# certfhe/CSGN

Hardware: NVIDIA B200
Metric: ctxt-mul+decrypt output blocks/s (higher is better)
Workload: dtype u64

## Files before the change

csgn_b200/_native.py:

```python
import ctypes
import os
import re
import warnings

from . import build as _build

_u64 = ctypes.c_uint64
_u64p = ctypes.POINTER(ctypes.c_uint64)
_vp = ctypes.c_void_p
_vpp = ctypes.POINTER(ctypes.c_void_p)

SIGNATURES = {
    "csgn_init": (ctypes.c_int, [ctypes.c_int]),
    "csgn_shutdown": (ctypes.c_int, []),
    "csgn_is_initialized": (ctypes.c_int, []),
    "csgn_last_error": (ctypes.c_char_p, []),
    "csgn_version": (ctypes.c_char_p, []),
    "csgn_device_info": (ctypes.c_int, [ctypes.POINTER(ctypes.c_int), _u64p, _u64p, ctypes.POINTER(ctypes.c_int)]),
    "csgn_set_stream": (ctypes.c_int, [_vp]),
    "csgn_get_stream": (_vp, []),
    "csgn_set_auto_lanes": (ctypes.c_int, [ctypes.c_int]),
    "csgn_get_auto_lanes": (ctypes.c_int, []),
    "csgn_sync": (ctypes.c_int, []),
    "csgn_launch_count": (_u64, []),
    "csgn_words_per_block": (ctypes.c_uint32, [_u64]),
    "csgn_host_alloc": (ctypes.c_int, [ctypes.c_size_t, _vpp]),
    "csgn_host_free": (ctypes.c_int, [_vp]),
    "csgn_buf_upload": (ctypes.c_int, [_vp, _u64, ctypes.c_uint32, _vpp]),
    "csgn_buf_upload_copy": (ctypes.c_int, [_vp, _u64, ctypes.c_uint32, _vpp]),
    "csgn_buf_upload_batch": (ctypes.c_int, [_vp, _vp, ctypes.c_uint32, ctypes.c_uint32, _vp]),
    "csgn_buf_free_batch": (ctypes.c_int, [_vp, ctypes.c_uint32]),
    "csgn_buf_alloc": (ctypes.c_int, [_u64, ctypes.c_uint32, _vpp]),
    "csgn_buf_wrap": (ctypes.c_int, [_vp, _u64, ctypes.c_uint32, _vpp]),
    "csgn_buf_clone": (ctypes.c_int, [_vp, _vpp]),
    "csgn_buf_download": (ctypes.c_int, [_vp, _vp]),
    "csgn_buf_download_range": (ctypes.c_int, [_vp, _u64, _u64, _vp]),
    "csgn_buf_slice": (ctypes.c_int, [_vp, _u64, _u64, _vpp]),
    "csgn_buf_free": (ctypes.c_int, [_vp]),
    "csgn_buf_blocks": (_u64, [_vp]),
    "csgn_buf_words_per_block": (ctypes.c_uint32, [_vp]),
    "csgn_buf_device_ptr": (_vp, [_vp]),
    "csgn_mul": (ctypes.c_int, [_vp, _vp, _vpp]),
    "csgn_mul_into": (ctypes.c_int, [_vp, _vp, _vp]),
    "csgn_concat": (ctypes.c_int, [_vp, _vp, _vpp]),
    "csgn_append": (ctypes.c_int, [_vp, _vp]),
    "csgn_concat_lazy": (ctypes.c_int, [_vp, _vp, _vpp]),
    "csgn_buf_segments": (ctypes.c_int, [_vp]),
    "csgn_buf_retained": (ctypes.c_int, [_vp]),
    "csgn_buf_flatten": (ctypes.c_int, [_vp]),
    "csgn_key_create": (ctypes.c_int, [_u64, _vp, ctypes.c_uint32, _vpp]),
    "csgn_key_free": (ctypes.c_int, [_vp]),
    "csgn_decrypt": (ctypes.c_int, [_vp, _vp, ctypes.POINTER(ctypes.c_uint8)]),
    "csgn_decrypt_count": (ctypes.c_int, [_vp, _vp, _u64p]),
    "csgn_decrypt_count_async": (ctypes.c_int, [_vp, _vp, _vp]),
    "csgn_decrypt_product": (ctypes.c_int, [ctypes.POINTER(_vp), ctypes.c_uint32, _vp, ctypes.POINTER(ctypes.c_uint8), _u64p]),
    "csgn_decrypt_deferred": (ctypes.c_int, [_vp, _vp, _vpp]),
    "csgn_result_ready": (ctypes.c_int, [_vp]),
    "csgn_result_wait": (ctypes.c_int, [_vp, _u64p]),
    "csgn_result_free": (ctypes.c_int, [_vp]),
    "csgn_mul_count_async": (ctypes.c_int, [_vp, _vp, _vp, _vpp, _vp]),
    "csgn_mul_decrypt": (ctypes.c_int, [_vp, _vp, _vp, _vpp, ctypes.POINTER(ctypes.c_uint8), _u64p]),
    "csgn_mul_count_batch_async": (ctypes.c_int, [ctypes.POINTER(_vp), ctypes.POINTER(_vp), ctypes.c_uint32, _vp,
                                                  ctypes.POINTER(_vp), _vp]),
    "csgn_mul_decrypt_deferred": (ctypes.c_int, [_vp, _vp, _vp, _vpp, _vpp]),
    "csgn_mul_decrypt_sharded_async": (ctypes.c_int, [_vp, _vp, _vp, _vpp, _vp, ctypes.c_uint32, ctypes.c_uint32, _vp, _vp]),
    "csgn_mul_decrypt_sharded_batch_async": (ctypes.c_int, [ctypes.POINTER(_vp), ctypes.POINTER(_vp), ctypes.c_uint32, _vp,
                                                            ctypes.POINTER(_vp), _vp, ctypes.c_uint32, _vp]),
    "csgn_mul_batch": (ctypes.c_int, [ctypes.POINTER(_vp), ctypes.POINTER(_vp), ctypes.c_uint32, ctypes.POINTER(_vp)]),
    "csgn_mul_into_batch": (ctypes.c_int, [ctypes.POINTER(_vp), ctypes.POINTER(_vp), ctypes.c_uint32, ctypes.POINTER(_vp)]),
    "csgn_decrypt_count_batch_async": (ctypes.c_int, [ctypes.POINTER(_vp), ctypes.c_uint32, _vp, _vp]),
    "csgn_decrypt_batch": (ctypes.c_int, [ctypes.POINTER(_vp), ctypes.c_uint32, _vp, ctypes.POINTER(ctypes.c_uint8), _u64p]),
    "csgn_decrypt_sharded_batch_async": (ctypes.c_int, [ctypes.POINTER(_vp), ctypes.c_uint32, _vp, _vp, ctypes.c_uint32, _vp]),
    "csgn_decrypt_positions": (ctypes.c_int, [_vp, _u64, _vp, ctypes.c_uint32, ctypes.POINTER(ctypes.c_uint8)]),
    "csgn_encrypt_batch": (ctypes.c_int, [_vp, _vp, _u64, _u64, _u64, _vpp]),
    "csgn_seg_mul": (ctypes.c_int, [_vp, _vp, _vp, _vp, _u64, _vp, _vpp]),
    "csgn_seg_concat": (ctypes.c_int, [_vp, _vp, _vp, _vp, _u64, _vp, _vpp]),
    "csgn_seg_mul_sum": (ctypes.c_int, [ctypes.POINTER(_vp), ctypes.POINTER(_vp), ctypes.POINTER(_vp), ctypes.POINTER(_vp),
                                        ctypes.c_uint32, ctypes.POINTER(_vp), ctypes.POINTER(_vp), ctypes.c_uint32, _u64,
                                        _vp, _vpp]),
    "csgn_seg_mul_sum_compact": (ctypes.c_int, [ctypes.POINTER(_vp), ctypes.POINTER(_vp), ctypes.POINTER(_vp),
                                                ctypes.POINTER(_vp), ctypes.c_uint32, ctypes.POINTER(_vp),
                                                ctypes.POINTER(_vp), ctypes.c_uint32, _u64, ctypes.c_uint32, _vp, _vpp]),
# ... 87 lines not shown
```

csgn_b200/certfhe/device_types.cpp:

```cpp
#include "certFHE.h"
#include "engine_glue.h"

#include <cstdlib>
#include <ctime>
#include <utility>
#include <vector>

namespace certFHE {

namespace glue {

void check(int status, const char *what) {
    if (status != CSGN_OK) throw Error(string(what) + ": " + csgn_last_error());
}

void ensure_engine() {
    if (csgn_is_initialized()) return;
    check(csgn_init(-1), "csgn_init");
    check(csgn_set_auto_lanes(Library::getAutoLanes() ? 1 : 0), "csgn_set_auto_lanes");
}

}

namespace {

inline uint64_t canonical_bits(uint64_t i, uint64_t L, uint64_t rem) {
    return ((i % L) + 1 == L && rem) ? rem : 64;
}

void require_canonical_bitlen(const uint64_t *bitlen, uint64_t len, const Context &ctx) {
    const uint64_t L = ctx.getDefaultN(), rem = ctx.getN() % 64;
    uint64_t diff = 0;
    const uint64_t head = len < L ? len : L;
    for (uint64_t k = 0; k < head; ++k) diff |= bitlen[k] ^ canonical_bits(k, L, rem);
    if (len > L && memcmp(bitlen + L, bitlen, (size_t)(len - L) * sizeof(uint64_t)) != 0) diff = 1;
    if (!diff) return;
    for (uint64_t i = 0; i < len; ++i)
        if (bitlen[i] != canonical_bits(i, L, rem))
            throw Error("Ciphertext: bitlen[" + to_string(i) + "] = " + to_string(bitlen[i]) +
                        " is not the canonical pattern for N = " + to_string(ctx.getN()) +
                        " (the reference would mis-index such an object, src/SecretKey.cpp:133)");
}

uint64_t *copy_words(const uint64_t *src, uint64_t n) {
    uint64_t *p = new uint64_t[n ? n : 1];
    if (n) memcpy(p, src, n * sizeof(uint64_t));
    return p;
}

}

namespace {

std::shared_ptr<csgn_buf> adopt(csgn_buf *b) {
    return std::shared_ptr<csgn_buf>(b, [](csgn_buf *p) { csgn_buf_free(p); });
}

}

Ciphertext::Ciphertext()
    : certFHEcontext(nullptr), host_v(nullptr), host_bitlen(nullptr), host_len(0), host_v_valid(false),
      staged(false), sharded(false) {}

Ciphertext::Ciphertext(const uint64_t *V, const uint64_t *Bitlen, const uint64_t len, const Context &context)
    : Ciphertext() {
    certFHEcontext = new Context(context);
    const uint64_t L = context.getDefaultN();
    if (L == 0 || len % L != 0)
        throw Error("Ciphertext: len = " + to_string(len) + " is not a multiple of the " + to_string(L) +
                    " words per block");
    if (Bitlen) require_canonical_bitlen(Bitlen, len, context);
    glue::ensure_engine();
    csgn_buf *b = nullptr;
    glue::check(csgn_buf_upload_copy(V, len / L, (uint32_t)L, &b), "csgn_buf_upload_copy");
    dev = adopt(b);
}

Ciphertext::Ciphertext(const Ciphertext &o) : Ciphertext() {
    if (o.certFHEcontext) certFHEcontext = new Context(*o.certFHEcontext);
    sharded = o.sharded;
    if (o.staged) {
        host_v = copy_words(o.host_v, o.host_len);
        if (o.host_bitlen) host_bitlen = copy_words(o.host_bitlen, o.host_len);
        host_len = o.host_len;
        host_v_valid = true;
        staged = true;
    } else {
        dev = o.dev;
        factors = o.factors;
        product_slot = o.product_slot;
    }
}

Ciphertext::Ciphertext(Ciphertext &&o) noexcept
    : dev(std::move(o.dev)), factors(std::move(o.factors)), product_slot(std::move(o.product_slot)),
      certFHEcontext(o.certFHEcontext), host_v(o.host_v),
      host_bitlen(o.host_bitlen), host_len(o.host_len), host_v_valid(o.host_v_valid), staged(o.staged),
      sharded(o.sharded) {
    o.factors.clear();
    o.product_slot.reset();
    o.certFHEcontext = nullptr;
    o.host_v = o.host_bitlen = nullptr;
    o.host_len = 0;
    o.host_v_valid = o.staged = false;
}

Ciphertext::~Ciphertext() {
    release();
    delete certFHEcontext;
    certFHEcontext = nullptr;
}

void Ciphertext::invalidate_mirror() const {
    delete[] host_v;
    delete[] host_bitlen;
    host_v = host_bitlen = nullptr;
    host_len = 0;
    host_v_valid = false;
}

void Ciphertext::release() {
    dev.reset();
    factors.clear();
    product_slot.reset();
    invalidate_mirror();
    staged = false;
}
// ... 652 lines not shown
```

csgn_b200/csrc/capi.cu:

```cuda
#include "capi_internal.cuh"

#include <atomic>
#include <cstdarg>
#if defined(__x86_64__) && !defined(__CUDA_ARCH__)
#include <emmintrin.h>
#define CSGN_HAVE_SSE2_STREAM 1
#endif

#ifdef CSGN_BUILD_VARIANTS
#define CSGN_VERSION_STRING "csgn-b200 0.2 (sm_100a) +variants"
#else
#define CSGN_VERSION_STRING "csgn-b200 0.2 (sm_100a)"
#endif

namespace csgn {
namespace detail {

State g;
DeviceProps g_props;
std::atomic<uint64_t> g_launches{0};
thread_local std::string t_error;

int fail(int code, const char *fmt, ...) {
    char buf[512];
    va_list ap;
    va_start(ap, fmt);
    vsnprintf(buf, sizeof buf, fmt, ap);
    va_end(ap);
    t_error = buf;
    return code;
}

int cuda_fail(cudaError_t e, const char *what) {
    cudaGetLastError();
    return fail(e == cudaErrorMemoryAllocation ? CSGN_ERR_OUT_OF_MEMORY : CSGN_ERR_CUDA, "%s: %s (%s)", what,
                cudaGetErrorString(e), cudaGetErrorName(e));
}

uint64_t *fold_scratch() {
    size_t i = 0;
    for (; i < g.scratch_streams.size(); ++i)
        if (g.scratch_streams[i] == g.stream) break;
    if (i == g.scratch_streams.size()) {
        if (i < kScratchSlots) {
            g.scratch_streams.push_back(g.stream);
        } else {
            i = kScratchSlots - 1;
            cudaDeviceSynchronize();
        }
    }
    return g.d_scratch + 8 + 2 * i;
}

bool folds_overlap() { return g.in_batch || g.auto_lanes; }

int dev_alloc(uint64_t words, uint64_t **out, cudaStream_t stream) {
    *out = nullptr;
    if (words == 0) return CSGN_OK;
    void *p = nullptr;
    cudaError_t e = cudaMallocAsync(&p, words * sizeof(uint64_t), stream ? stream : g.stream);
// ... 207 lines not shown
    for (csgn_buf *x : segs) csgn_buf_free(x);
}

int need_dense(const csgn_buf *b) {
    if (!is_rope(b)) return CSGN_OK;
    csgn_buf *m = const_cast<csgn_buf *>(b);
    uint64_t *d = nullptr;
    const uint64_t words = b->n_blocks * b->L;
    int rc = dev_alloc(words, &d);
    if (rc != CSGN_OK) return rc;
    rc = copy_words_into(b, d);
    if (rc != CSGN_OK) {
        dev_free(d);
        return rc;
    }
    m->d = d;
    m->cap_words = words;
    m->owns = true;
    m->writer = {g.stream, g.tick++};
    m->readers.clear();
    drop_segments(b);
    return CSGN_OK;
}

}

using namespace detail;

const DeviceProps &device_props() { return g_props; }
void set_device_props(const DeviceProps &p) { g_props = p; }
void count_launch(unsigned n) { g_launches.fetch_add(n, std::memory_order_relaxed); }
uint64_t launches() { return g_launches.load(std::memory_order_relaxed); }

static bool g_tuning = true;

long env_long(const char *name, long dflt) {
    if (!g_tuning) return dflt;
    const char *s = std::getenv(name);
    if (!s || !*s) return dflt;
    char *end = nullptr;
    long v = std::strtol(s, &end, 10);
    return (end && *end == 0) ? v : dflt;
}

}

namespace {
struct StagingSlot {
    void *p;
    size_t cap;
    cudaEvent_t done;
};
std::vector<StagingSlot> g_staging;
size_t g_staging_bytes = 0;
constexpr size_t kStagingMaxTotal = 512ull << 20, kStagingMaxOne = 64ull << 20;

StagingSlot *take_staging(size_t bytes) {
    StagingSlot *best = nullptr;
    for (StagingSlot &sl : g_staging) {
        if (sl.cap < bytes || (best && best->cap <= sl.cap)) continue;
        if (cudaEventQuery(sl.done) != cudaSuccess) {
            cudaGetLastError();
            continue;
        }
        best = &sl;
    }
    if (best) return best;
    size_t cap = 64 << 10;
    while (cap < bytes) cap <<= 1;
    if (g_staging_bytes + cap > kStagingMaxTotal) return nullptr;
    StagingSlot sl = {nullptr, cap, nullptr};
    if (cudaHostAlloc(&sl.p, cap, cudaHostAllocDefault) != cudaSuccess) {
        cudaGetLastError();
        return nullptr;
    }
    if (cudaEventCreateWithFlags(&sl.done, cudaEventDisableTiming) != cudaSuccess) {
        cudaGetLastError();
        cudaFreeHost(sl.p);
        return nullptr;
    }
    g_staging.push_back(sl);
    g_staging_bytes += cap;
    return &g_staging.back();
}
}

using namespace csgn;
using namespace csgn::detail;

extern "C" {

int csgn_init(int device) {
    csgn::g_tuning = true;
    if (device < 0) device = (int)env_long("CSGN_DEVICE", env_long("LOCAL_RANK", 0));
    csgn::g_tuning = std::getenv("CSGN_TUNING") != nullptr;
    if (g.inited) {
        if (g.device == device) return CSGN_OK;
        return fail(CSGN_ERR_INVALID_ARGUMENT, "already bound to device %d (one process per GPU)", g.device);
    }
    int n = 0;
    cudaError_t e = cudaGetDeviceCount(&n);
    if (e != cudaSuccess || n == 0) {
        cudaGetLastError();
        return fail(CSGN_ERR_NO_DEVICE, "no CUDA device visible (%s); this engine has no CPU path",
                    e == cudaSuccess ? "count = 0" : cudaGetErrorString(e));
    }
    if (device >= n) return fail(CSGN_ERR_NO_DEVICE, "device %d requested, %d visible", device, n);
    CU(cudaSetDevice(device));
    cudaDeviceProp p;
    CU(cudaGetDeviceProperties(&p, device));
    if (p.major != 10)
        return fail(CSGN_ERR_NO_DEVICE, "device %d is sm_%d%d; the kernels are built for sm_100a (B200) only",
                    device, p.major, p.minor);
    DeviceProps dp;
    dp.device = device;
    dp.sm_count = p.multiProcessorCount;
    dp.cc = p.major * 10 + p.minor;
    dp.smem_optin = p.sharedMemPerBlockOptin;
    set_device_props(dp);

    CU(cudaStreamCreateWithFlags(&g.own_stream, cudaStreamNonBlocking));
    g.stream = g.own_stream;
    CU(cudaStreamCreateWithFlags(&g.copy_stream, cudaStreamNonBlocking));
    {
        const char *e = std::getenv("CSGN_LANES");
        g.n_lanes = e && *e ? std::max(1, std::min((int)State::kMaxLanes, std::atoi(e))) : 2;
    }
    for (int i = 0; i < g.n_lanes; ++i) {
        CU(cudaStreamCreateWithFlags(&g.lane[i], cudaStreamNonBlocking));
        CU(cudaEventCreateWithFlags(&g.lane_done[i], cudaEventDisableTiming));
    }
    CU(cudaEventCreateWithFlags(&g.fork_point, cudaEventDisableTiming));
    cudaMemPool_t pool;
    CU(cudaDeviceGetDefaultMemPool(&pool, device));
    uint64_t keep = UINT64_MAX;
    CU(cudaMemPoolSetAttribute(pool, cudaMemPoolAttrReleaseThreshold, &keep));
    int off = 0;
    CU(cudaMemPoolSetAttribute(pool, cudaMemPoolReuseAllowInternalDependencies, &off));
    CU(cudaMalloc(reinterpret_cast<void **>(&g.d_scratch), (8 + 2 * kScratchSlots) * sizeof(uint64_t)));
    CU(cudaMemset(g.d_scratch, 0, (8 + 2 * kScratchSlots) * sizeof(uint64_t)));
    CU(cudaHostAlloc(reinterpret_cast<void **>(&g.h_result), 8 * sizeof(uint64_t), cudaHostAllocDefault));
    CU(cudaMalloc(reinterpret_cast<void **>(&g.d_results), kResultSlots * sizeof(uint64_t)));
    CU(cudaHostAlloc(reinterpret_cast<void **>(&g.h_results), kResultSlots * sizeof(uint64_t), cudaHostAllocDefault));
    g.free_results.clear();
    for (uint32_t i = kResultSlots; i > 0; --i) g.free_results.push_back(i - 1);
    {
        const char *e = std::getenv("CSGN_AUTO_LANES");
        g.auto_lanes = e && *e && std::atoi(e) != 0;
    }
    g.device = device;
    g.inited = true;
    return CSGN_OK;
}

int csgn_shutdown(void) {
    if (!g.inited) return CSGN_OK;
    cudaSetDevice(g.device);
    cudaDeviceSynchronize();
    for (const State::UploadSlot &sl : g.upload_cache) {
        cudaFreeAsync(sl.d, g.stream);
        cudaEventDestroy(sl.freed);
    }
    cudaStreamSynchronize(g.stream);
    for (StagingSlot &sl : g_staging) {
        cudaFreeHost(sl.p);
        cudaEventDestroy(sl.done);
    }
    g_staging.clear();
    g_staging_bytes = 0;
    cudaFree(g.d_scratch);
    cudaFreeHost(g.h_result);
    if (g.d_results) cudaFree(g.d_results);
    if (g.h_results) cudaFreeHost(g.h_results);
    for (cudaEvent_t e : g.event_pool) cudaEventDestroy(e);
    for (int i = 0; i < State::kMaxLanes; ++i) {
        if (g.lane[i]) {
            cudaStreamSynchronize(g.lane[i]);
            cudaStreamDestroy(g.lane[i]);
        }
        if (g.lane_done[i]) cudaEventDestroy(g.lane_done[i]);
    }
    if (g.fork_point) cudaEventDestroy(g.fork_point);
    cudaStreamDestroy(g.copy_stream);
    cudaStreamDestroy(g.own_stream);
    g = State();
    return CSGN_OK;
}

int csgn_is_initialized(void) { return g.inited ? 1 : 0; }
const char *csgn_last_error(void) { return t_error.c_str(); }
const char *csgn_version(void) { return CSGN_VERSION_STRING; }

int csgn_device_info(int *sm_count, uint64_t *hbm_total, uint64_t *hbm_free, int *cc) {
    NEED_INIT();
    size_t fr = 0, tot = 0;
    CU(cudaMemGetInfo(&fr, &tot));
    if (sm_count) *sm_count = device_props().sm_count;
    if (hbm_total) *hbm_total = tot;
    if (hbm_free) *hbm_free = fr;
    if (cc) *cc = device_props().cc;
    return CSGN_OK;
}

int csgn_set_stream(void *cuda_stream) {
    NEED_INIT();
    g.stream = cuda_stream ? static_cast<cudaStream_t>(cuda_stream) : g.own_stream;
    return CSGN_OK;
}

int csgn_set_auto_lanes(int on) {
    NEED_INIT();
    g.auto_lanes = on != 0;
    return CSGN_OK;
}

int csgn_get_auto_lanes(void) { return g.inited && g.auto_lanes ? 1 : 0; }

void *csgn_get_stream(void) { return g.inited ? static_cast<void *>(g.stream) : nullptr; }

int csgn_sync(void) {
    NEED_INIT();
    CU(cudaStreamSynchronize(g.copy_stream));
// ... 17 lines not shown
    CU(cudaHostAlloc(out, bytes ? bytes : 1, cudaHostAllocDefault));
    return CSGN_OK;
}

int csgn_host_free(void *p) {
    NEED_INIT();
    if (p) CU(cudaFreeHost(p));
    return CSGN_OK;
}

int csgn_buf_alloc(uint64_t n_blocks, uint32_t L, csgn_buf **out) {
    NEED_INIT();
    if (!out) return fail(CSGN_ERR_INVALID_ARGUMENT, "null output handle");
    return new_buf(n_blocks, L, 0, out);
}

int csgn_buf_upload(const uint64_t *host_words, uint64_t n_blocks, uint32_t L, csgn_buf **out) {
    NEED_INIT();
    if (!out) return fail(CSGN_ERR_INVALID_ARGUMENT, "null output handle");
    if (n_blocks && !host_words) return fail(CSGN_ERR_INVALID_ARGUMENT, "null host words");
    if (L == 0) return fail(CSGN_ERR_INVALID_ARGUMENT, "words per block must be > 0");
    csgn_buf *b = nullptr;
    uint64_t cap = 0;
    uint64_t *cached = (n_blocks && n_blocks <= kUploadCacheMaxWords / L) ? take_upload_slot(n_blocks * L, &cap) : nullptr;
    if (cached) {
        b = new csgn_buf;
        b->d = cached;
        b->n_blocks = n_blocks;
        b->L = L;
        b->cap_words = cap;
        b->writer = {g.copy_stream, g.tick++};
    } else {
        int rc = new_buf(n_blocks, L, 0, &b, g.copy_stream);
        if (rc != CSGN_OK) return rc;
    }
    b->recycle = true;
    if (n_blocks) {
        cudaError_t e = cudaMemcpyAsync(b->d, host_words, n_blocks * L * sizeof(uint64_t), cudaMemcpyHostToDevice,
                                        g.copy_stream);
        if (e == cudaSuccess) {
            b->ready = take_event();
            e = b->ready ? cudaEventRecord(b->ready, g.copy_stream) : cudaStreamSynchronize(g.copy_stream);
            if (e == cudaSuccess) b->writer = StreamMark();
        }
        if (e != cudaSuccess) {
            csgn_buf_free(b);
            return cuda_fail(e, "cudaMemcpyAsync(H2D)");
        }
    }
    *out = b;
    return CSGN_OK;
}

namespace {
void copy_to_staging(void *dst, const void *src, size_t bytes) {
#ifdef CSGN_HAVE_SSE2_STREAM
    if (bytes >= (32u << 10)) {
        char *d = static_cast<char *>(dst);
        const char *s = static_cast<const char *>(src);
        size_t head = (16u - (reinterpret_cast<uintptr_t>(d) & 15u)) & 15u;
        memcpy(d, s, head);
        d += head, s += head, bytes -= head;
        const size_t n = bytes / 64;
        for (size_t i = 0; i < n; ++i, s += 64, d += 64) {
            const __m128i a = _mm_loadu_si128(reinterpret_cast<const __m128i *>(s));
            const __m128i b = _mm_loadu_si128(reinterpret_cast<const __m128i *>(s + 16));
            const __m128i c = _mm_loadu_si128(reinterpret_cast<const __m128i *>(s + 32));
            const __m128i e = _mm_loadu_si128(reinterpret_cast<const __m128i *>(s + 48));
            _mm_stream_si128(reinterpret_cast<__m128i *>(d), a);
            _mm_stream_si128(reinterpret_cast<__m128i *>(d + 16), b);
            _mm_stream_si128(reinterpret_cast<__m128i *>(d + 32), c);
            _mm_stream_si128(reinterpret_cast<__m128i *>(d + 48), e);
        }
        memcpy(d, s, bytes - n * 64);
        _mm_sfence();
        return;
    }
#endif
    memcpy(dst, src, bytes);
}
}

}

namespace csgn {
namespace detail {

int stage_into(void *d, const void *host, size_t bytes) {
    if (bytes == 0) return CSGN_OK;
    StagingSlot *sl = bytes <= kStagingMaxOne ? take_staging(bytes) : nullptr;
    cudaError_t e;
    if (sl) {
        copy_to_staging(sl->p, host, bytes);
        e = cudaMemcpyAsync(d, sl->p, bytes, cudaMemcpyHostToDevice, g.stream);
        cudaEventRecord(sl->done, g.stream);
    } else {
        e = cudaMemcpyAsync(d, host, bytes, cudaMemcpyHostToDevice, g.stream);
        if (e == cudaSuccess) e = cudaStreamSynchronize(g.stream);
        if (e == cudaSuccess) note_synced(g.stream);
    }
    return e == cudaSuccess ? CSGN_OK : cuda_fail(e, "table upload");
}

int stage_to_device(const void *host, size_t bytes, void **out) {
    *out = nullptr;
    if (bytes == 0) return CSGN_OK;
    uint64_t *d = nullptr;
    int rc = dev_alloc((bytes + 7) / 8, &d);
    if (rc != CSGN_OK) return rc;
    rc = stage_into(d, host, bytes);
    if (rc != CSGN_OK) {
        dev_free(d);
        return rc;
    }
    *out = d;
    return CSGN_OK;
}

int read_back(void *host, const void *d, size_t bytes) {
    if (bytes == 0) return CSGN_OK;
    StagingSlot *sl = bytes <= kStagingMaxOne ? take_staging(bytes) : nullptr;
    cudaError_t e = cudaMemcpyAsync(sl ? sl->p : host, d, bytes, cudaMemcpyDeviceToHost, g.stream);
    if (e == cudaSuccess && sl) e = cudaEventRecord(sl->done, g.stream);
    if (e == cudaSuccess) e = cudaStreamSynchronize(g.stream);
    if (e != cudaSuccess) return cuda_fail(e, "table read-back");
    note_synced(g.stream);
    if (sl) memcpy(host, sl->p, bytes);
    return CSGN_OK;
}

}
}

extern "C" {

int csgn_buf_upload_copy(const uint64_t *host_words, uint64_t n_blocks, uint32_t L, csgn_buf **out) {
    NEED_INIT();
    if (L == 0) return fail(CSGN_ERR_INVALID_ARGUMENT, "words per block must be > 0");
    if (n_blocks > (UINT64_MAX / 8) / L) return fail(CSGN_ERR_INVALID_ARGUMENT, "block count overflows");
    const size_t bytes = (size_t)n_blocks * L * sizeof(uint64_t);
    StagingSlot *sl = (bytes && bytes <= kStagingMaxOne && host_words) ? take_staging(bytes) : nullptr;
    if (!sl) {
        int rc = csgn_buf_upload(host_words, n_blocks, L, out);
        if (rc != CSGN_OK) return rc;
        CU(cudaStreamSynchronize(g.copy_stream));
        note_synced(g.copy_stream);
        return CSGN_OK;
    }
    copy_to_staging(sl->p, host_words, bytes);
    int rc = csgn_buf_upload(static_cast<const uint64_t *>(sl->p), n_blocks, L, out);
    cudaEventRecord(sl->done, g.copy_stream);
    return rc;
}

int csgn_buf_upload_batch(const uint64_t *const *host_words, const uint64_t *n_blocks, uint32_t n, uint32_t L,
                          csgn_buf **out) {
    NEED_INIT();
    if (n == 0) return CSGN_OK;
    if (!host_words || !n_blocks || !out) return fail(CSGN_ERR_INVALID_ARGUMENT, "null argument");
    if (L == 0) return fail(CSGN_ERR_INVALID_ARGUMENT, "words per block must be > 0");
    constexpr uint64_t kAlignWords = 32;
    std::vector<uint64_t> off(n);
    uint64_t total = 0;
    for (uint32_t i = 0; i < n; ++i) {
        if (n_blocks[i] && !host_words[i]) return fail(CSGN_ERR_INVALID_ARGUMENT, "null host words (operand %u)", i);
        if (n_blocks[i] > (UINT64_MAX / 16) / L) return fail(CSGN_ERR_INVALID_ARGUMENT, "block count overflows");
        off[i] = total;
        total += (n_blocks[i] * L + kAlignWords - 1) / kAlignWords * kAlignWords;
    }
    if (total == 0) total = kAlignWords;
    csgn_slab *sl = new csgn_slab;
    uint64_t cap = 0;
    sl->d = total <= kUploadCacheMaxWords ? take_upload_slot(total, &cap) : nullptr;
    if (sl->d) sl->cap_words = cap;
    else {
        int rc = dev_alloc(total, &sl->d, g.copy_stream);
        if (rc != CSGN_OK) {
            delete sl;
            return rc;
        }
        sl->cap_words = total;
    }
    std::vector<void *> dsts, srcs;
    std::vector<size_t> sizes;
    for (uint32_t i = 0; i < n; ++i)
        if (n_blocks[i]) {
            dsts.push_back(sl->d + off[i]);
            srcs.push_back(const_cast<uint64_t *>(host_words[i]));
            sizes.push_back((size_t)n_blocks[i] * L * sizeof(uint64_t));
        }
    cudaError_t e = cudaSuccess;
    for (size_t i = 0; i < dsts.size() && e == cudaSuccess;) {
        size_t j = i + 1, bytes = sizes[i];
        while (j < dsts.size() && static_cast<char *>(srcs[i]) + bytes == static_cast<char *>(srcs[j]) &&
               static_cast<char *>(dsts[i]) + bytes == static_cast<char *>(dsts[j])) {
            bytes += sizes[j];
            ++j;
        }
        e = cudaMemcpyAsync(dsts[i], srcs[i], bytes, cudaMemcpyHostToDevice, g.copy_stream);
        i = j;
    }
    if (e != cudaSuccess) {
        cudaStreamSynchronize(g.copy_stream);
        dev_free(sl->d);
        delete sl;
// ... 986 lines not shown
```

csgn_b200/csrc/capi_internal.cuh:

```cuda
#pragma once

#include "../../include/csgn.h"

#include <cuda_runtime.h>

#include <algorithm>
#include <cstdint>
#include <cstdio>
#include <cstdlib>
#include <cstring>
#include <string>
#include <vector>

#include "kernels.cuh"

struct StreamMark {
    cudaStream_t s = nullptr;
    uint64_t tick = 0;
};

struct csgn_slab {
    uint64_t *d = nullptr;
    uint64_t cap_words = 0;
    uint32_t refs = 0;
// ... 79 lines not shown
    uint64_t *d_scratch = nullptr;
    uint64_t *h_result = nullptr;
    std::vector<cudaStream_t> scratch_streams;
    uint64_t tick = 1;
    std::vector<StreamMark> synced;
    struct Waited {
        cudaStream_t consumer, producer;
        uint64_t tick;
    };
    std::vector<Waited> waited;
    bool auto_lanes = false;
    bool in_batch = false;
    bool in_auto = false;
    uint32_t rr = 0;
    uint64_t *h_results = nullptr, *d_results = nullptr;
    std::vector<uint32_t> free_results;
};
extern State g;
constexpr uint32_t kResultSlots = 4096;
constexpr uint32_t kScratchSlots = 256;

int fail(int code, const char *fmt, ...);
int cuda_fail(cudaError_t e, const char *what);

#define CU(call)                                            \
    do {                                                    \
        cudaError_t e_ = (call);                            \
        if (e_ != cudaSuccess) return cuda_fail(e_, #call); \
    } while (0)

#define NEED_INIT()                                                                              \
    do {                                                                                         \
        if (!g.inited) return fail(CSGN_ERR_NOT_INITIALIZED, "csgn_init has not been called");   \
        int cur_ = -1;                                                                           \
        if (cudaGetDevice(&cur_) != cudaSuccess || cur_ != g.device) CU(cudaSetDevice(g.device)); \
    } while (0)

int dev_alloc(uint64_t words, uint64_t **out, cudaStream_t stream = nullptr);
void dev_free(void *p);
cudaEvent_t take_event();
void acquire_read(const csgn_buf *b);
void acquire_write(const csgn_buf *b);
void note_synced(cudaStream_t s);
int new_buf(uint64_t n_blocks, uint32_t L, uint64_t cap_words, csgn_buf **out, cudaStream_t stream = nullptr);
int need_dense(const csgn_buf *b);
inline bool is_rope(const csgn_buf *b) { return b && !b->segs.empty(); }
uint64_t *fold_scratch();
bool folds_overlap();

int stage_to_device(const void *host, size_t bytes, void **out);
int stage_into(void *d, const void *host, size_t bytes);
int read_back(void *host, const void *d, size_t bytes);

struct LaneScope {
    cudaStream_t home;
    int used = 1;
    bool active;
    bool was_in_batch;
    explicit LaneScope(uint32_t n_items) : home(g.stream), active(g.n_lanes > 1 && n_items > 1), was_in_batch(g.in_batch) {
        g.in_batch = true;
        if (!active) return;
        used = (int)std::min<uint32_t>(n_items, (uint32_t)g.n_lanes);
        cudaEventRecord(g.fork_point, home);
        for (int i = 1; i < used; ++i) cudaStreamWaitEvent(g.lane[i], g.fork_point, 0);
    }
    void enter(uint32_t item) {
        if (!active) return;
        const uint32_t way = item % (uint32_t)used;
        g.stream = way == 0 ? home : g.lane[way];
    }
    void join() {
        g.in_batch = was_in_batch;
        if (!active) return;
        g.stream = home;
        for (int i = 1; i < used; ++i) {
            cudaEventRecord(g.lane_done[i], g.lane[i]);
            cudaStreamWaitEvent(home, g.lane_done[i], 0);
        }
        active = false;
    }
    ~LaneScope() { join(); }
};

int check_mul_operands(const csgn_buf *a, const csgn_buf *b);
int check_mul_out(const csgn_buf *a, const csgn_buf *b, const csgn_buf *out);
int check_key(const csgn_buf *a, const csgn_key *key);
int fused_out(const csgn_buf *a, const csgn_buf *b, csgn_buf **out, csgn_buf **dst, bool *allocated);
int enqueue_mul(const csgn_buf *a, const csgn_buf *b, csgn_buf *out, const csgn_key *key, uint64_t *device_count,
                const csgn::PeerPush *pp);

struct AutoLane {
    cudaStream_t home;
    bool active = false;
    AutoLane(const csgn_buf *x, const csgn_buf *y = nullptr);
    ~AutoLane() {
        if (active) {
            g.stream = home;
            g.in_auto = false;
        }
    }
};

}
}
```

include/csgn.h:

```cpp
#ifndef CSGN_H_
#define CSGN_H_

#include <stddef.h>
#include <stdint.h>

#ifdef __cplusplus
extern "C" {
#endif

typedef enum csgn_status {
    CSGN_OK = 0,
    CSGN_ERR_NOT_INITIALIZED = -1,
    CSGN_ERR_INVALID_ARGUMENT = -2,
    CSGN_ERR_CUDA = -3,
    CSGN_ERR_NO_DEVICE = -4,
    CSGN_ERR_SHAPE_MISMATCH = -5,
    CSGN_ERR_OUT_OF_MEMORY = -6,
    CSGN_ERR_TIMEOUT = -7
} csgn_status;

typedef struct csgn_buf csgn_buf;
typedef struct csgn_key csgn_key;
typedef struct csgn_perm csgn_perm;


int csgn_init(int device);
int csgn_shutdown(void);
int csgn_is_initialized(void);
const char *csgn_last_error(void);
const char *csgn_version(void);
int csgn_device_info(int *sm_count, uint64_t *hbm_total, uint64_t *hbm_free, int *cc);
int csgn_set_stream(void *cuda_stream);
void *csgn_get_stream(void);
int csgn_set_auto_lanes(int on);
int csgn_get_auto_lanes(void);
int csgn_sync(void);
uint64_t csgn_launch_count(void);

uint32_t csgn_words_per_block(uint64_t N);

int csgn_host_alloc(size_t bytes, void **out);
int csgn_host_free(void *p);


int csgn_buf_upload(const uint64_t *host_words, uint64_t n_blocks, uint32_t L, csgn_buf **out);
int csgn_buf_upload_copy(const uint64_t *host_words, uint64_t n_blocks, uint32_t L, csgn_buf **out);
int csgn_buf_upload_batch(const uint64_t *const *host_words, const uint64_t *n_blocks, uint32_t n, uint32_t L,
                          csgn_buf **out);
int csgn_buf_free_batch(csgn_buf *const *bufs, uint32_t n);
int csgn_buf_alloc(uint64_t n_blocks, uint32_t L, csgn_buf **out);
int csgn_buf_wrap(void *device_words, uint64_t n_blocks, uint32_t L, csgn_buf **out);
int csgn_buf_clone(const csgn_buf *src, csgn_buf **out);
int csgn_buf_download(const csgn_buf *buf, uint64_t *host_words);
int csgn_buf_download_range(const csgn_buf *buf, uint64_t first_block, uint64_t n_blocks,
                            uint64_t *host_words);
int csgn_buf_slice(const csgn_buf *src, uint64_t first_block, uint64_t n_blocks, csgn_buf **out);
int csgn_buf_free(csgn_buf *buf);
uint64_t csgn_buf_blocks(const csgn_buf *buf);
uint32_t csgn_buf_words_per_block(const csgn_buf *buf);
void *csgn_buf_device_ptr(const csgn_buf *buf);


int csgn_mul(const csgn_buf *a, const csgn_buf *b, csgn_buf **out);
int csgn_mul_into(const csgn_buf *a, const csgn_buf *b, csgn_buf *out);

int csgn_concat(const csgn_buf *a, const csgn_buf *b, csgn_buf **out);
int csgn_append(csgn_buf *a, const csgn_buf *b);
int csgn_concat_lazy(const csgn_buf *a, const csgn_buf *b, csgn_buf **out);
int csgn_buf_segments(const csgn_buf *buf);
int csgn_buf_retained(const csgn_buf *buf);
int csgn_buf_flatten(csgn_buf *buf);

int csgn_key_create(uint64_t N, const uint64_t *positions, uint32_t D, csgn_key **out);
int csgn_key_free(csgn_key *key);

int csgn_decrypt(const csgn_buf *c, const csgn_key *key, uint8_t *bit);
int csgn_decrypt_count(const csgn_buf *c, const csgn_key *key, uint64_t *count);
int csgn_decrypt_count_async(const csgn_buf *c, const csgn_key *key, uint64_t *device_count);
int csgn_decrypt_product(const csgn_buf *const *factors, uint32_t n_factors, const csgn_key *key, uint8_t *bit,
                         uint64_t *count);
typedef struct csgn_result csgn_result;
int csgn_decrypt_deferred(const csgn_buf *c, const csgn_key *key, csgn_result **out);
int csgn_result_ready(const csgn_result *r);
int csgn_result_wait(csgn_result *r, uint64_t *count);
int csgn_result_free(csgn_result *r);

int csgn_mul_count_async(const csgn_buf *a, const csgn_buf *b, const csgn_key *key, csgn_buf **out, uint64_t *device_count);
int csgn_mul_decrypt(const csgn_buf *a, const csgn_buf *b, const csgn_key *key, csgn_buf **out, uint8_t *bit,
                     uint64_t *count);
int csgn_mul_count_batch_async(const csgn_buf *const *a, const csgn_buf *const *b, uint32_t n, const csgn_key *key,
                               csgn_buf **out, uint64_t *device_counts);
int csgn_mul_decrypt_deferred(const csgn_buf *a, const csgn_buf *b, const csgn_key *key, csgn_buf **prod,
                              csgn_result **out);

int csgn_mul_batch(const csgn_buf *const *a, const csgn_buf *const *b, uint32_t n, csgn_buf **out);
int csgn_mul_into_batch(const csgn_buf *const *a, const csgn_buf *const *b, uint32_t n, csgn_buf *const *out);
int csgn_decrypt_count_batch_async(const csgn_buf *const *c, uint32_t n, const csgn_key *key, uint64_t *device_counts);
int csgn_decrypt_batch(const csgn_buf *const *c, uint32_t n, const csgn_key *key, uint8_t *bits, uint64_t *counts);

// ... 76 lines not shown
```

Before: 44.25 billion.

## Parallelize host staging copy and fuse bitlen validation into multithreaded copy

Replaces the single-threaded streaming memcpy into pinned staging buffers with a persistent spin/sleep worker pool that splits large copies into chunks, and fuses the canonical-Bitlen check into the same chunked pass instead of a separate host scan before upload. Staging slot selection now prefers exact-size slots round-robin. This targets host-side ciphertext ingest cost, at the price of extra threads, spinning CPU time, and more complex synchronization.

```diff
diff --git a/csgn_b200/_native.py b/csgn_b200/_native.py
--- a/csgn_b200/_native.py
+++ b/csgn_b200/_native.py
@@ -28,6 +28,9 @@
     "csgn_host_free": (ctypes.c_int, [_vp]),
     "csgn_buf_upload": (ctypes.c_int, [_vp, _u64, ctypes.c_uint32, _vpp]),
     "csgn_buf_upload_copy": (ctypes.c_int, [_vp, _u64, ctypes.c_uint32, _vpp]),
+    "csgn_buf_upload_copy_checked": (ctypes.c_int, [_vp, _vp, _u64, ctypes.c_uint32, _u64, _vpp]),
+    "csgn_host_copy_checked": (ctypes.c_int, [_vp, _vp, _vp, _u64, ctypes.c_uint32, _u64, ctypes.c_int]),
+    "csgn_copy_threads": (ctypes.c_int, []),
     "csgn_buf_upload_batch": (ctypes.c_int, [_vp, _vp, ctypes.c_uint32, ctypes.c_uint32, _vp]),
     "csgn_buf_free_batch": (ctypes.c_int, [_vp, ctypes.c_uint32]),
     "csgn_buf_alloc": (ctypes.c_int, [_u64, ctypes.c_uint32, _vpp]),
diff --git a/csgn_b200/certfhe/device_types.cpp b/csgn_b200/certfhe/device_types.cpp
--- a/csgn_b200/certfhe/device_types.cpp
+++ b/csgn_b200/certfhe/device_types.cpp
@@ -69,10 +69,15 @@
     if (L == 0 || len % L != 0)
         throw Error("Ciphertext: len = " + to_string(len) + " is not a multiple of the " + to_string(L) +
                     " words per block");
-    if (Bitlen) require_canonical_bitlen(Bitlen, len, context);
     glue::ensure_engine();
     csgn_buf *b = nullptr;
-    glue::check(csgn_buf_upload_copy(V, len / L, (uint32_t)L, &b), "csgn_buf_upload_copy");
+    if (Bitlen) {
+        const int rc = csgn_buf_upload_copy_checked(V, Bitlen, len / L, (uint32_t)L, context.getN(), &b);
+        if (rc == CSGN_ERR_INVALID_ARGUMENT) require_canonical_bitlen(Bitlen, len, context);
+        glue::check(rc, "csgn_buf_upload_copy_checked");
+    } else {
+        glue::check(csgn_buf_upload_copy(V, len / L, (uint32_t)L, &b), "csgn_buf_upload_copy");
+    }
     dev = adopt(b);
 }
 
diff --git a/csgn_b200/csrc/capi.cu b/csgn_b200/csrc/capi.cu
--- a/csgn_b200/csrc/capi.cu
+++ b/csgn_b200/csrc/capi.cu
@@ -2,10 +2,6 @@
 
 #include <atomic>
 #include <cstdarg>
-#if defined(__x86_64__) && !defined(__CUDA_ARCH__)
-#include <emmintrin.h>
-#define CSGN_HAVE_SSE2_STREAM 1
-#endif
 
 #ifdef CSGN_BUILD_VARIANTS
 #define CSGN_VERSION_STRING "csgn-b200 0.2 (sm_100a) +variants"
@@ -319,22 +315,31 @@
     cudaEvent_t done;
 };
 std::vector<StagingSlot> g_staging;
-size_t g_staging_bytes = 0;
+size_t g_staging_bytes = 0, g_staging_next = 0;
 constexpr size_t kStagingMaxTotal = 512ull << 20, kStagingMaxOne = 64ull << 20;
 
+bool staging_free(const StagingSlot &sl) {
+    if (cudaEventQuery(sl.done) == cudaSuccess) return true;
+    cudaGetLastError();
+    return false;
+}
+
 StagingSlot *take_staging(size_t bytes) {
+    size_t cap = 64 << 10;
+    while (cap < bytes) cap <<= 1;
+    const size_t n = g_staging.size();
+    for (size_t k = 0; k < n; ++k) {
+        const size_t i = (g_staging_next + k) % n;
+        if (g_staging[i].cap != cap || !staging_free(g_staging[i])) continue;
+        g_staging_next = i + 1;
+        return &g_staging[i];
+    }
     StagingSlot *best = nullptr;
     for (StagingSlot &sl : g_staging) {
-        if (sl.cap < bytes || (best && best->cap <= sl.cap)) continue;
-        if (cudaEventQuery(sl.done) != cudaSuccess) {
-            cudaGetLastError();
-            continue;
-        }
-        best = &sl;
+        if (sl.cap < bytes || sl.cap == cap || (best && best->cap <= sl.cap)) continue;
+        if (staging_free(sl)) best = &sl;
     }
     if (best) return best;
-    size_t cap = 64 << 10;
-    while (cap < bytes) cap <<= 1;
     if (g_staging_bytes + cap > kStagingMaxTotal) return nullptr;
     StagingSlot sl = {nullptr, cap, nullptr};
     if (cudaHostAlloc(&sl.p, cap, cudaHostAllocDefault) != cudaSuccess) {
@@ -348,6 +353,7 @@
     }
     g_staging.push_back(sl);
     g_staging_bytes += cap;
+    g_staging_next = g_staging.size();
     return &g_staging.back();
 }
 }
@@ -421,6 +427,7 @@
 }
 
 int csgn_shutdown(void) {
+    stop_copy_workers();
     if (!g.inited) return CSGN_OK;
     cudaSetDevice(g.device);
     cudaDeviceSynchronize();
@@ -434,7 +441,7 @@
         cudaEventDestroy(sl.done);
     }
     g_staging.clear();
-    g_staging_bytes = 0;
+    g_staging_bytes = g_staging_next = 0;
     cudaFree(g.d_scratch);
     cudaFreeHost(g.h_result);
     if (g.d_results) cudaFree(g.d_results);
@@ -558,35 +565,6 @@
     return CSGN_OK;
 }
 
-namespace {
-void copy_to_staging(void *dst, const void *src, size_t bytes) {
-#ifdef CSGN_HAVE_SSE2_STREAM
-    if (bytes >= (32u << 10)) {
-        char *d = static_cast<char *>(dst);
-        const char *s = static_cast<const char *>(src);
-        size_t head = (16u - (reinterpret_cast<uintptr_t>(d) & 15u)) & 15u;
-        memcpy(d, s, head);
-        d += head, s += head, bytes -= head;
-        const size_t n = bytes / 64;
-        for (size_t i = 0; i < n; ++i, s += 64, d += 64) {
-            const __m128i a = _mm_loadu_si128(reinterpret_cast<const __m128i *>(s));
-            const __m128i b = _mm_loadu_si128(reinterpret_cast<const __m128i *>(s + 16));
-            const __m128i c = _mm_loadu_si128(reinterpret_cast<const __m128i *>(s + 32));
-            const __m128i e = _mm_loadu_si128(reinterpret_cast<const __m128i *>(s + 48));
-            _mm_stream_si128(reinterpret_cast<__m128i *>(d), a);
-            _mm_stream_si128(reinterpret_cast<__m128i *>(d + 16), b);
-            _mm_stream_si128(reinterpret_cast<__m128i *>(d + 32), c);
-            _mm_stream_si128(reinterpret_cast<__m128i *>(d + 48), e);
-        }
-        memcpy(d, s, bytes - n * 64);
-        _mm_sfence();
-        return;
-    }
-#endif
-    memcpy(dst, src, bytes);
-}
-}
-
 }
 
 namespace csgn {
@@ -597,7 +575,7 @@
     StagingSlot *sl = bytes <= kStagingMaxOne ? take_staging(bytes) : nullptr;
     cudaError_t e;
     if (sl) {
-        copy_to_staging(sl->p, host, bytes);
+        staging_copy(sl->p, host, bytes, nullptr, 1, 0, 0);
         e = cudaMemcpyAsync(d, sl->p, bytes, cudaMemcpyHostToDevice, g.stream);
         cudaEventRecord(sl->done, g.stream);
     } else {
@@ -638,14 +616,23 @@
 }
 }
 
-extern "C" {
-
-int csgn_buf_upload_copy(const uint64_t *host_words, uint64_t n_blocks, uint32_t L, csgn_buf **out) {
-    NEED_INIT();
+namespace {
+
+int bitlen_mismatch(const uint64_t *bitlen, uint32_t L, uint64_t N) {
+    uint64_t i = 0;
+    while (bitlen[i] == canonical_bitlen_word(i, L, N % 64)) ++i;
+    return fail(CSGN_ERR_INVALID_ARGUMENT, "bitlen[%llu] = %llu is not the canonical pattern for N = %llu",
+                (unsigned long long)i, (unsigned long long)bitlen[i], (unsigned long long)N);
+}
+
+int upload_copy(const uint64_t *host_words, const uint64_t *bitlen, uint64_t n_blocks, uint32_t L, uint64_t N,
+                csgn_buf **out) {
     if (L == 0) return fail(CSGN_ERR_INVALID_ARGUMENT, "words per block must be > 0");
     if (n_blocks > (UINT64_MAX / 8) / L) return fail(CSGN_ERR_INVALID_ARGUMENT, "block count overflows");
     const size_t bytes = (size_t)n_blocks * L * sizeof(uint64_t);
     StagingSlot *sl = (bytes && bytes <= kStagingMaxOne && host_words) ? take_staging(bytes) : nullptr;
+    if (!staging_copy(sl ? sl->p : nullptr, host_words, (sl || bitlen) ? bytes : 0, bitlen, L, N % 64))
+        return bitlen_mismatch(bitlen, L, N);
     if (!sl) {
         int rc = csgn_buf_upload(host_words, n_blocks, L, out);
         if (rc != CSGN_OK) return rc;
@@ -653,10 +640,49 @@
         note_synced(g.copy_stream);
         return CSGN_OK;
     }
-    copy_to_staging(sl->p, host_words, bytes);
     int rc = csgn_buf_upload(static_cast<const uint64_t *>(sl->p), n_blocks, L, out);
     cudaEventRecord(sl->done, g.copy_stream);
     return rc;
+}
+
+int check_bitlen_args(const uint64_t *bitlen, uint64_t n_blocks, uint32_t L, uint64_t N) {
+    if (n_blocks && !bitlen) return fail(CSGN_ERR_INVALID_ARGUMENT, "null Bitlen");
+    if (N == 0 || csgn_words_per_block(N) != L)
+        return fail(CSGN_ERR_INVALID_ARGUMENT, "%u words per block do not hold N = %llu bits", L, (unsigned long long)N);
+    return CSGN_OK;
+}
+
+}
+
+extern "C" {
+
+int csgn_buf_upload_copy(const uint64_t *host_words, uint64_t n_blocks, uint32_t L, csgn_buf **out) {
+    NEED_INIT();
+    return upload_copy(host_words, nullptr, n_blocks, L, 0, out);
+}
+
+int csgn_buf_upload_copy_checked(const uint64_t *host_words, const uint64_t *bitlen, uint64_t n_blocks, uint32_t L,
+                                 uint64_t N, csgn_buf **out) {
+    NEED_INIT();
+    const int rc = check_bitlen_args(bitlen, n_blocks, L, N);
+    return rc != CSGN_OK ? rc : upload_copy(host_words, bitlen, n_blocks, L, N, out);
+}
+
+int csgn_copy_threads(void) { return copy_threads(); }
+
+int csgn_host_copy_checked(uint64_t *dst, const uint64_t *host_words, const uint64_t *bitlen, uint64_t n_blocks,
+                           uint32_t L, uint64_t N, int threads) {
+    if (L == 0) return fail(CSGN_ERR_INVALID_ARGUMENT, "words per block must be > 0");
+    if (n_blocks > (UINT64_MAX / 8) / L) return fail(CSGN_ERR_INVALID_ARGUMENT, "block count overflows");
+    if (n_blocks && (!dst || !host_words)) return fail(CSGN_ERR_INVALID_ARGUMENT, "null words");
+    if (bitlen) {
+        const int rc = check_bitlen_args(bitlen, n_blocks, L, N);
+        if (rc != CSGN_OK) return rc;
+    }
+    if (!staging_copy(dst, host_words, (size_t)n_blocks * L * sizeof(uint64_t), bitlen, L, N % 64,
+                      std::min(threads, kMaxCopyThreads)))
+        return bitlen_mismatch(bitlen, L, N);
+    return CSGN_OK;
 }
 
 int csgn_buf_upload_batch(const uint64_t *const *host_words, const uint64_t *n_blocks, uint32_t n, uint32_t L,
diff --git a/csgn_b200/csrc/capi_internal.cuh b/csgn_b200/csrc/capi_internal.cuh
--- a/csgn_b200/csrc/capi_internal.cuh
+++ b/csgn_b200/csrc/capi_internal.cuh
@@ -155,6 +155,17 @@
 int stage_into(void *d, const void *host, size_t bytes);
 int read_back(void *host, const void *d, size_t bytes);
 
+inline uint64_t canonical_bitlen_word(uint64_t i, uint64_t L, uint64_t rem) {
+    return ((i % L) + 1 == L && rem) ? rem : 64;
+}
+constexpr size_t kParallelCopyMin = 64u << 10;
+constexpr int kMaxCopyThreads = 16;
+constexpr int kDefaultCopyThreads = 4;
+bool staging_copy(void *dst, const void *src, size_t bytes, const uint64_t *bitlen, uint64_t L, uint64_t rem,
+                  int threads = 0);
+int copy_threads();
+void stop_copy_workers();
+
 struct LaneScope {
     cudaStream_t home;
     int used = 1;
diff --git a/csgn_b200/csrc/host_copy.cu b/csgn_b200/csrc/host_copy.cu
--- /dev/null
+++ b/csgn_b200/csrc/host_copy.cu
@@ -0,0 +1,215 @@
+#include "capi_internal.cuh"
+
+#include <atomic>
+#include <chrono>
+#include <condition_variable>
+#include <cstring>
+#include <mutex>
+#include <new>
+#include <pthread.h>
+#include <thread>
+#if defined(__x86_64__) && !defined(__CUDA_ARCH__)
+#include <emmintrin.h>
+#include <immintrin.h>
+#define CSGN_HAVE_SSE2_STREAM 1
+#endif
+
+namespace csgn {
+namespace detail {
+
+namespace {
+
+constexpr size_t kChunkMin = 16u << 10;
+constexpr auto kSpin = std::chrono::microseconds(50);
+
+inline void cpu_relax() {
+#ifdef CSGN_HAVE_SSE2_STREAM
+    _mm_pause();
+#endif
+}
+
+inline void store_fence() {
+#ifdef CSGN_HAVE_SSE2_STREAM
+    _mm_sfence();
+#endif
+}
+
+void stream_copy(void *dst, const void *src, size_t bytes) {
+#ifdef CSGN_HAVE_SSE2_STREAM
+    char *d = static_cast<char *>(dst);
+    const char *s = static_cast<const char *>(src);
+    size_t head = (16u - (reinterpret_cast<uintptr_t>(d) & 15u)) & 15u;
+    if (head > bytes) head = bytes;
+    memcpy(d, s, head);
+    d += head, s += head, bytes -= head;
+    const size_t n = bytes / 64;
+    for (size_t i = 0; i < n; ++i, s += 64, d += 64) {
+        const __m128i a = _mm_loadu_si128(reinterpret_cast<const __m128i *>(s));
+        const __m128i b = _mm_loadu_si128(reinterpret_cast<const __m128i *>(s + 16));
+        const __m128i c = _mm_loadu_si128(reinterpret_cast<const __m128i *>(s + 32));
+        const __m128i e = _mm_loadu_si128(reinterpret_cast<const __m128i *>(s + 48));
+        _mm_stream_si128(reinterpret_cast<__m128i *>(d), a);
+        _mm_stream_si128(reinterpret_cast<__m128i *>(d + 16), b);
+        _mm_stream_si128(reinterpret_cast<__m128i *>(d + 32), c);
+        _mm_stream_si128(reinterpret_cast<__m128i *>(d + 48), e);
+    }
+    memcpy(d, s, bytes - n * 64);
+#else
+    memcpy(dst, src, bytes);
+#endif
+}
+
+bool canonical_slice(const uint64_t *bitlen, uint64_t w0, uint64_t n, uint64_t L, uint64_t rem) {
+    const uint64_t head = n < L ? n : L;
+    uint64_t diff = 0;
+    for (uint64_t k = 0; k < head; ++k) diff |= bitlen[w0 + k] ^ canonical_bitlen_word(w0 + k, L, rem);
+    if (diff) return false;
+    return n <= L || memcmp(bitlen + w0 + L, bitlen + w0, (size_t)(n - L) * sizeof(uint64_t)) == 0;
+}
+
+class CopyPool {
+  public:
+    ~CopyPool() { stop(); }
+
+    bool run(char *dst, const char *src, size_t bytes, const uint64_t *bitlen, uint64_t L, uint64_t rem, int threads) {
+        resize(threads - 1);
+        size_t chunk = (bytes + 2 * threads - 1) / (2 * threads);
+        if (chunk < kChunkMin) chunk = kChunkMin;
+        chunk = (chunk + 63) & ~size_t(63);
+        dst_ = dst, src_ = src, bytes_ = bytes, chunk_ = chunk, bitlen_ = bitlen, L_ = L, rem_ = rem;
+        const uint32_t n_chunks = (uint32_t)((bytes + chunk - 1) / chunk);
+        n_chunks_.store(n_chunks, std::memory_order_relaxed);
+        bad_.store(false, std::memory_order_relaxed);
+        done_.store(0, std::memory_order_relaxed);
+        const uint32_t gen = ++gen_;
+        claim_.store((uint64_t)gen << 32, std::memory_order_seq_cst);
+        if (sleepers_.load(std::memory_order_seq_cst) > 0) {
+            std::lock_guard<std::mutex> lk(mu_);
+            cv_.notify_all();
+        }
+        work(gen);
+        while (done_.load(std::memory_order_acquire) < n_chunks) cpu_relax();
+        return !bad_.load(std::memory_order_relaxed);
+    }
+
+    void stop() { resize(0); }
+
+    void forget_workers() {
+        new (&workers_) std::vector<std::thread>();
+        new (&mu_) std::mutex();
+        new (&cv_) std::condition_variable();
+        sleepers_.store(0);
+        quit_.store(false);
+    }
+
+  private:
+    void resize(int n) {
+        if (n < 0) n = 0;
+        if ((size_t)n == workers_.size()) return;
+        if (!workers_.empty()) {
+            {
+                std::lock_guard<std::mutex> lk(mu_);
+                quit_.store(true, std::memory_order_seq_cst);
+                cv_.notify_all();
+            }
+            for (std::thread &t : workers_) t.join();
+            workers_.clear();
+            quit_.store(false);
+        }
+        for (int i = 0; i < n; ++i) workers_.emplace_back([this] { loop(); });
+    }
+
+    void work(uint32_t gen) {
+        for (;;) {
+            uint64_t c = claim_.load(std::memory_order_acquire);
+            do {
+                if ((uint32_t)(c >> 32) != gen || (uint32_t)c >= n_chunks_.load(std::memory_order_relaxed)) return;
+            } while (!claim_.compare_exchange_weak(c, c + 1, std::memory_order_acq_rel));
+            const size_t off = (size_t)(uint32_t)c * chunk_;
+            const size_t len = std::min(chunk_, bytes_ - off);
+            if (bitlen_ && !canonical_slice(bitlen_, off / 8, len / 8, L_, rem_)) bad_.store(true, std::memory_order_relaxed);
+            if (dst_) {
+                stream_copy(dst_ + off, src_ + off, len);
+                store_fence();
+            }
+            done_.fetch_add(1, std::memory_order_release);
+        }
+    }
+
+    void loop() {
+        uint32_t seen = (uint32_t)(claim_.load(std::memory_order_acquire) >> 32);
+        for (;;) {
+            auto t0 = std::chrono::steady_clock::now();
+            uint32_t spins = 0;
+            uint32_t gen;
+            while ((gen = (uint32_t)(claim_.load(std::memory_order_acquire) >> 32)) == seen) {
+                if (quit_.load(std::memory_order_relaxed)) return;
+                cpu_relax();
+                if (++spins % 256 || std::chrono::steady_clock::now() - t0 < kSpin) continue;
+                std::unique_lock<std::mutex> lk(mu_);
+                sleepers_.fetch_add(1, std::memory_order_seq_cst);
+                cv_.wait(lk, [&] {
+                    return quit_.load(std::memory_order_seq_cst) ||
+                           (uint32_t)(claim_.load(std::memory_order_seq_cst) >> 32) != seen;
+                });
+                sleepers_.fetch_sub(1, std::memory_order_seq_cst);
+                t0 = std::chrono::steady_clock::now();
+            }
+            seen = gen;
+            work(gen);
+        }
+    }
+
+    std::vector<std::thread> workers_;
+    std::mutex mu_;
+    std::condition_variable cv_;
+    std::atomic<uint64_t> claim_{0};
+    std::atomic<uint32_t> done_{0};
+    std::atomic<int> sleepers_{0};
+    std::atomic<bool> bad_{false}, quit_{false};
+    uint32_t gen_ = 0;
+    char *dst_ = nullptr;
+    const char *src_ = nullptr;
+    size_t bytes_ = 0, chunk_ = 0;
+    std::atomic<uint32_t> n_chunks_{0};
+    const uint64_t *bitlen_ = nullptr;
+    uint64_t L_ = 1, rem_ = 0;
+};
+
+CopyPool g_pool;
+const int g_atfork = pthread_atfork(nullptr, nullptr, [] { g_pool.forget_workers(); });
+
+}
+
+int copy_threads() {
+    static const int n = [] {
+        const char *e = std::getenv("CSGN_COPY_THREADS");
+        if (e && *e) return std::max(1, std::min(kMaxCopyThreads, std::atoi(e)));
+        const int cores = (int)std::thread::hardware_concurrency();
+        return std::max(1, std::min(kDefaultCopyThreads, cores / 4));
+    }();
+    return n;
+}
+
+void stop_copy_workers() { g_pool.stop(); }
+
+bool staging_copy(void *dst, const void *src, size_t bytes, const uint64_t *bitlen, uint64_t L, uint64_t rem,
+                  int threads) {
+    if (threads <= 0) threads = copy_threads();
+    if (threads > 1 && bytes >= kParallelCopyMin)
+        return g_pool.run(static_cast<char *>(dst), static_cast<const char *>(src), bytes, bitlen, L, rem, threads);
+    if (bitlen && !canonical_slice(bitlen, 0, bytes / 8, L, rem)) return false;
+    if (!dst) return true;
+#ifdef CSGN_HAVE_SSE2_STREAM
+    if (bytes >= (32u << 10)) {
+        stream_copy(dst, src, bytes);
+        store_fence();
+        return true;
+    }
+#endif
+    memcpy(dst, src, bytes);
+    return true;
+}
+
+}
+}
diff --git a/include/csgn.h b/include/csgn.h
--- a/include/csgn.h
+++ b/include/csgn.h
@@ -45,6 +45,11 @@
 
 int csgn_buf_upload(const uint64_t *host_words, uint64_t n_blocks, uint32_t L, csgn_buf **out);
 int csgn_buf_upload_copy(const uint64_t *host_words, uint64_t n_blocks, uint32_t L, csgn_buf **out);
+int csgn_buf_upload_copy_checked(const uint64_t *host_words, const uint64_t *bitlen, uint64_t n_blocks, uint32_t L,
+                                 uint64_t N, csgn_buf **out);
+int csgn_host_copy_checked(uint64_t *dst, const uint64_t *host_words, const uint64_t *bitlen, uint64_t n_blocks,
+                           uint32_t L, uint64_t N, int threads);
+int csgn_copy_threads(void);
 int csgn_buf_upload_batch(const uint64_t *const *host_words, const uint64_t *n_blocks, uint32_t n, uint32_t L,
                           csgn_buf **out);
 int csgn_buf_free_batch(csgn_buf *const *bufs, uint32_t n);
```

Result: no change. 44.34 billion, median of 6 (+0.2%).
